# Zanue/EndoDAV

Hardware: AMD Instinct MI355X
Metric: depth frames/sec (518x518, T=8 clip) (higher is better)
Workload: dtype f32

## Files before the change

endodav_amd/csrc/conv_dma.hip:

```cpp
#include <atomic>
#include <cstdlib>
#include <type_traits>

#include "gemm_common.hpp"

namespace edv {
namespace {

constexpr int CBK = 32;
__device__ __attribute__((aligned(256))) float g_zero_page[64];

template <int WGM, int EP, bool SPLIT, bool BUF>
__global__ __launch_bounds__(256, 4) void conv3_dma_kernel(const GemmDesc g, const GemmSplit sp) {
    constexpr int WGN = 4 / WGM;
    constexpr int BM = 32 * WGM, BN = 32 * WGN;
    constexpr int IA = BM / 32, IB = BN / 32;
    constexpr int STAGE = (BM + BN) * CBK;
    __shared__ __attribute__((aligned(16))) float smem[2 * STAGE];
    const int tid = threadIdx.x, lane = tid & 63, wave = tid >> 6, l31 = lane & 31, lh = lane >> 5;
    const int wave_s = __builtin_amdgcn_readfirstlane(wave);
    const bool prelu = g.pre_relu != 0;
    const int wm = wave / WGN, wn = wave % WGN;
    const int tiles_n = (g.N + BN - 1) / BN;
    const int bid = xcd_remap(blockIdx.x, gridDim.x);
    const unsigned a_bytes = BUF ? (unsigned)((g.M > 0 ? ((g.M - 1) / (g.cOH * g.cOW) + 1) : 0) * (long long)g.cH * g.cW * g.cC * 4) : 0u;
    const auto rA = __builtin_amdgcn_make_buffer_rsrc(const_cast<float *>(g.A), 0, a_bytes, 0x00020000);
    const auto rW = __builtin_amdgcn_make_buffer_rsrc(const_cast<float *>(g.W), 0, 0xffffffff, 0x00020000);
    const int srow = lane >> 3, spos = lane & 7;
    const float *zero = g_zero_page + spos * 4;
    const int opix = g.cOH * g.cOW;
    const int nkt = g.K / CBK;
    const int ra = wm * 32 + l31, rb = wn * 32 + l31;
    const int swa = (ra >> 1) & 7, swb = (rb >> 1) & 7;

    long long u = SPLIT ? (long long)bid * sp.chunk : 0;
    const long long u_end = SPLIT ? (u + sp.chunk < sp.units ? u + sp.chunk : sp.units) : 0;
    bool once = true;
    for (;;) {
        int tile, kt0, kt1, lt = 0;
        float *part = nullptr;
        if (SPLIT) {
            if (u >= u_end) break;
            lt = (int)(u / nkt);
            kt0 = (int)(u - (long long)lt * nkt);
            const long long left = u_end - u;
            kt1 = kt0 + left < nkt ? kt0 + (int)left : nkt;
            tile = lt;
            if (!(kt0 == 0 && kt1 == nkt)) part = split_slot<SPLIT_SLOT>(sp, bid, u);
            u += kt1 - kt0;
        } else {
            if (!once) break;
            once = false;
            tile = bid;
            kt0 = 0;
            kt1 = nkt;
        }
        const int tm = tile / tiles_n, tn = tile - tm * tiles_n;
        const long long m0 = (long long)tm * BM;
        const int n0 = tn * BN;

        const float *pa[IA];
        unsigned va[IA], vb[IB];
        int okmask[IA];
#pragma unroll
        for (int i = 0; i < IA; ++i) {
            const int r = (BM / 4) * wave + 8 * i + srow;
            const int c = spos ^ ((r >> 1) & 7);
            long long m = m0 + r;
            m = m < g.M ? m : g.M - 1;
            const long long f = BUF ? (long long)((unsigned)m / (unsigned)opix) : m / opix;
            const int p = BUF ? (int)((unsigned)m - (unsigned)f * (unsigned)opix) : (int)(m - f * opix);
            const int oy = p / g.cOW, ox = p - oy * g.cOW;
            const int iy0 = oy * g.cS - 1, ix0 = ox * g.cS - 1;
            pa[i] = g.A + ((f * g.cH + iy0) * (long long)g.cW + ix0) * g.cC + c * 4;
            va[i] = (unsigned)((((f * g.cH + iy0 + 1) * (long long)g.cW + ix0 + 1) * g.cC + c * 4) * 4);
            int mk = 0;
#pragma unroll
            for (int d = 0; d < 3; ++d) {
                if (iy0 + d >= 0 && iy0 + d < g.cH) mk |= 1 << d;
                if (ix0 + d >= 0 && ix0 + d < g.cW) mk |= 8 << d;
            }
            okmask[i] = mk;
        }
        const float *pb[IB];
#pragma unroll
        for (int i = 0; i < IB; ++i) {
            const int r = (BN / 4) * wave + 8 * i + srow;
            const int c = spos ^ ((r >> 1) & 7);
            int n = n0 + r;
            n = n < g.N ? n : g.N - 1;
            pb[i] = g.W + (long long)n * g.ldw + c * 4;
            vb[i] = (unsigned)(((long long)n * g.ldw + c * 4) * 4);
        }
        int n_c0, n_dy, n_dx;
        {
            const int k = kt0 * CBK, tap = k / g.cC;
            n_c0 = k - tap * g.cC;
            n_dy = tap / 3;
            n_dx = tap - n_dy * 3;
        }
        auto issue = [&](int kt, int st) {
            float *sA = smem + st * STAGE, *sB = sA + BM * CBK;
            const int k = kt * CBK;
            const int dy = n_dy, dx = n_dx, c0 = n_c0;
            n_c0 += CBK;
            if (n_c0 == g.cC) {
                n_c0 = 0;
                if (++n_dx == 3) {
                    n_dx = 0;
                    ++n_dy;
                }
            }
            const long long off = ((long long)dy * g.cW + dx) * g.cC + c0;
            const int need = (1 << dy) | (8 << dx);
#pragma unroll
            for (int i = 0; i < IA; ++i) {
                if constexpr (BUF) {
                    const int delta = (((dy - 1) * g.cW + (dx - 1)) * g.cC) * 4;
                    const unsigned vo = (okmask[i] & need) == need ? va[i] + (unsigned)delta : 0x80000000u + a_bytes;
                    __builtin_amdgcn_raw_ptr_buffer_load_lds(rA, (__attribute__((address_space(3))) void *)(sA + ((BM / 4) * wave_s + 8 * i) * CBK), 16, (unsigned)vo,
                                                             (int)(c0 * 4), 0, 0);
                } else {
                    const float *src = (okmask[i] & need) == need ? pa[i] + off : zero;
                    __builtin_amdgcn_global_load_lds((const __attribute__((address_space(1))) void *)src,
                                                     (__attribute__((address_space(3))) void *)(sA + ((BM / 4) * wave + 8 * i) * CBK), 16, 0, 0);
                }
            }
#pragma unroll
            for (int i = 0; i < IB; ++i) {
                if constexpr (BUF)
                    __builtin_amdgcn_raw_ptr_buffer_load_lds(rW, (__attribute__((address_space(3))) void *)(sB + ((BN / 4) * wave_s + 8 * i) * CBK), 16, (unsigned)vb[i], (int)(k * 4), 0,
                                                             0);
                else
                    __builtin_amdgcn_global_load_lds((const __attribute__((address_space(1))) void *)(pb[i] + k),
                                                     (__attribute__((address_space(3))) void *)(sB + ((BN / 4) * wave + 8 * i) * CBK), 16, 0, 0);
            }
        };
        const float *fpa[4], *fpb[4];
#pragma unroll
        for (int q = 0; q < 4; ++q) {
            fpa[q] = smem + ra * CBK + (((2 * q + lh) ^ swa) << 2);
            fpb[q] = smem + BM * CBK + rb * CBK + (((2 * q + lh) ^ swb) << 2);
        }

        EpiCols<1> cols;
        if (EP != 0) cols = gemm_epilogue_prefetch<1>(g, n0, wn * 32, l31);
        float w2v = 0.f, b2v = 0.f;
        if constexpr (EP >= 8) {
            w2v = g.w2[n0 + l31 < g.N ? n0 + l31 : g.N - 1];
            if (g.b2) b2v = g.b2[0];
        }
        f32x16 acc[1][1];
        auto epilogue = [&]() {
            if constexpr (EP >= 8) {
                static_assert(EP < 8 || (WGM == 4 && BUF && !SPLIT), "the fused 1x1 needs every column of a row in one wave, and 32-bit offsets");
                gemm_epilogue_dot<EP - 8>(g, acc[0][0], cols, w2v, b2v, m0 + wave_s * 32, n0, l31, lh);
            } else if constexpr (BUF && EP >= 1 && EP <= 3)
                gemm_epilogue_buf<EP - 1>(g, acc[0][0], cols, m0 + (wave_s / WGN) * 32, n0 + (wave_s % WGN) * 32, l31, lh);
            else
                gemm_epilogue_ep<1, 1, STORE_ROWS, EP>(g, acc, cols, m0, n0, wm * 32, wn * 32, l31, lh);
        };
#pragma unroll
        for (int r = 0; r < 16; ++r) acc[0][0][r] = 0.f;

        issue(kt0, 0);
        asm volatile("s_waitcnt vmcnt(0)" ::: "memory");
        __builtin_amdgcn_s_barrier();
        auto ktile = [&](int kt, auto st_tag) {
            constexpr int ST = decltype(st_tag)::value;
            if (kt + 1 < kt1) issue(kt + 1, ST ^ 1);
            f32x4 fa[4], fb[4];
#pragma unroll
            for (int q = 0; q < 4; ++q) {
                fa[q] = *reinterpret_cast<const f32x4 *>(fpa[q] + ST * STAGE);
                fb[q] = *reinterpret_cast<const f32x4 *>(fpb[q] + ST * STAGE);
            }
            __builtin_amdgcn_sched_barrier(0);
            if (prelu) {
#pragma unroll
                for (int q = 0; q < 4; ++q)
#pragma unroll
                    for (int e = 0; e < 4; ++e) fa[q][e] = __builtin_amdgcn_fmed3f(fa[q][e], 0.f, __builtin_inff());
            }
#pragma unroll
            for (int q = 0; q < 4; ++q) {
#pragma unroll
                for (int e = 0; e < 4; ++e) acc[0][0] = __builtin_amdgcn_mfma_f32_32x32x2f32(fa[q][e], fb[q][e], acc[0][0], 0, 0, 0);
            }
            __builtin_amdgcn_sched_barrier(0);
            asm volatile("s_waitcnt vmcnt(0)" ::: "memory");
            asm volatile("s_waitcnt lgkmcnt(0)" ::: "memory");
            __builtin_amdgcn_s_barrier();
        };
        {
            int kt = kt0;
            for (; kt + 1 < kt1; kt += 2) {
                ktile(kt, std::integral_constant<int, 0>{});
                ktile(kt + 1, std::integral_constant<int, 1>{});
            }
            if (kt < kt1) ktile(kt, std::integral_constant<int, 0>{});
        }
        if (SPLIT && part) {
#pragma unroll
            for (int r = 0; r < 16; ++r) __hip_atomic_store(&part[(wave * 16 + r) * 64 + lane], acc[0][0][r], __ATOMIC_RELAXED, __HIP_MEMORY_SCOPE_AGENT);
            const long long ub = (long long)lt * nkt;
            int g0, g1;
            const bool last = split_handoff(sp, &sp.cnt[lt], ub, nkt, reinterpret_cast<int *>(smem), tid, g0, g1);
            if (last) {
#pragma unroll
                for (int r = 0; r < 16; ++r) acc[0][0][r] = 0.f;
                const float *base = sp.ws + (wave * 16) * 64 + lane;
                int gg = g0;
                for (; gg + 1 <= g1; gg += 2) {
                    const float *qa = split_piece<SPLIT_SLOT>(base, sp, gg, ub);
                    const float *qb = split_piece<SPLIT_SLOT>(base, sp, gg + 1, ub);
                    float ta[16], tb[16];
#pragma unroll
                    for (int r = 0; r < 16; ++r) {
                        ta[r] = __hip_atomic_load(qa + r * 64, __ATOMIC_RELAXED, __HIP_MEMORY_SCOPE_AGENT);
                        tb[r] = __hip_atomic_load(qb + r * 64, __ATOMIC_RELAXED, __HIP_MEMORY_SCOPE_AGENT);
                    }
#pragma unroll
                    for (int r = 0; r < 16; ++r) acc[0][0][r] = (acc[0][0][r] + ta[r]) + tb[r];
                }
                if (gg <= g1) {
                    const float *qa = split_piece<SPLIT_SLOT>(base, sp, gg, ub);
#pragma unroll
                    for (int r = 0; r < 16; ++r) acc[0][0][r] += __hip_atomic_load(qa + r * 64, __ATOMIC_RELAXED, __HIP_MEMORY_SCOPE_AGENT);
                }
                epilogue();
            }
        } else {
            epilogue();
        }
    }
}

template <int WGM, int EP, bool SPLIT>
void launch_variant(const GemmDesc &d, const GemmSplit &sp, bool buf, unsigned grid, hipStream_t st) {
    if (buf) EDV_LAUNCH((conv3_dma_kernel<WGM, EP, SPLIT, true>), dim3(grid), dim3(256), 0, st, d, sp);
    else EDV_LAUNCH((conv3_dma_kernel<WGM, EP, SPLIT, false>), dim3(grid), dim3(256), 0, st, d, sp);
}

template <int WGM, int EP>
int conv_slots() {
    static DeviceSlotCache cache;
    return resident_workgroups(cache, (const void *)conv3_dma_kernel<WGM, EP, true, true>, 256, 0, 4, nullptr, nullptr);
}

template <int WGM, int EP>
int launch_conv_ep(const GemmDesc &d, long long tiles, hipStream_t st) {
    static const bool split_on = env_int("EDV_CONV_SPLIT", 1) != 0;
    static const bool buf_off = env_int("EDV_CONV_BUF", 1) == 0;
    const long long frames = (d.M - 1) / ((long long)d.cOH * d.cOW) + 1;
    const long long ld_out = std::max(std::max(d.ldc, d.R1 ? d.ldr1 : 0), d.R2 ? d.ldr2 : 0);
    const bool buf = !buf_off && frames * d.cH * d.cW * d.cC * 4 < (1ll << 31) - (1 << 20) && (long long)d.N * d.ldw * 4 < (1ll << 32) - (1 << 20) &&
                     (d.M + 64) * ld_out * 4 < (1ll << 32) - 4096;
    const SplitPolicy &pol = conv_dma_split_policy();
    GemmSplit sp{};
    long long grid;
    plan_plain(tiles, pol, &sp, &grid);
    if (split_on && d.ws && plan_split(tiles, conv_slots<WGM, EP>(), d.K / CBK, pol, &sp, &grid)) {
        split_bind(&sp, d.ws, pol);
        if (split_ws_floats(sp, pol) <= d.ws_floats && (uintptr_t)d.ws % 16 == 0) {
            launch_variant<WGM, EP, true>(d, sp, buf, (unsigned)grid, st);
            EDV_LAUNCH_OK();
            return 0;
        }
        grid = tiles;
    }
    launch_variant<WGM, EP, false>(d, sp, buf, (unsigned)grid, st);
    EDV_LAUNCH_OK();
    return 0;
}

template <int WGM>
int launch_conv(const GemmDesc &d, hipStream_t st) {
    constexpr int BM = 32 * WGM, BN = 32 * (4 / WGM);
    const long long tiles = ((d.M + BM - 1) / BM) * (long long)((d.N + BN - 1) / BN);
    EDV_CHECK(tiles > 0 && tiles < (1ll << 31), "bad grid");
    switch (epilogue_kind(d)) {
        case 1: return launch_conv_ep<WGM, 1>(d, tiles, st);
        case 3: return launch_conv_ep<WGM, 3>(d, tiles, st);
        default: return launch_conv_ep<WGM, 0>(d, tiles, st);
    }
}

std::atomic<int> g_conv_impl{0};

bool dot_fits_buffer(const GemmDesc &d) {
    const long long frames = (d.M - 1) / ((long long)d.cOH * d.cOW) + 1;
    return frames * d.cH * d.cW * d.cC * 4 < (1ll << 31) - (1 << 20) && (long long)d.N * d.ldw * 4 < (1ll << 32) - (1 << 20) && (d.M + 128) * 4 < (1ll << 32) - (1 << 20);
}

template <int EP>
int launch_conv_dot(const GemmDesc &d, hipStream_t st) {
    const long long tiles = (d.M + 127) / 128;
    EDV_CHECK(tiles > 0 && tiles < (1ll << 31), "bad grid");
    GemmSplit sp{};
    long long grid;
    plan_plain(tiles, conv_dma_split_policy(), &sp, &grid);
    EDV_LAUNCH((conv3_dma_kernel<4, EP, false, true>), dim3((unsigned)grid), dim3(256), 0, st, d, sp);
    EDV_LAUNCH_OK();
    return 0;
}

}

void set_conv_impl(int mode) { g_conv_impl.store(mode < 0 || mode > 2 ? 0 : mode, std::memory_order_relaxed); }
int conv_impl() { return g_conv_impl.load(std::memory_order_relaxed); }
bool conv_dot_enabled() {
    return conv_impl() != 1 && env_int("EDV_CONV_DOT", 1) != 0;
}

const SplitPolicy &conv_dma_split_policy() {
    static const SplitPolicy p{.min_kt = 18, .min_tiles = 16, .max_rounds = 0, .widen = false, .counters = SPLIT_MAX_COUNTERS, .slot_floats = SPLIT_SLOT,
                               .whole_rounds = false, .deep_kt = 48, .idle_factor = 8};
    return p;
}

bool conv_dma_supported(const GemmDesc &d) {
    return d.loader == LOAD_CONV3 && d.store == STORE_ROWS && d.cC % CBK == 0 && d.K == 9 * d.cC && d.ldw % 4 == 0 && d.M > 0 && d.N > 0;
}

bool conv_dot_supported(const GemmDesc &d) {
    return conv_dma_supported(d) && d.N <= 32 && (d.act == ACT_NONE || d.act == ACT_RELU) && d.act2 != ACT_GELU && d.act2 >= ACT_NONE && d.act2 <= ACT_SIGMOID_NEG &&
           !d.gamma && !d.R1 && !d.R2 && !d.P1 && d.c_map.period == 0 && dot_fits_buffer(d);
}

int conv_dot(const GemmDesc &d, hipStream_t st) {
    EDV_CHECK(d.A && d.W && d.w2 && d.dot_out, "null operand");
    EDV_CHECK(conv_dot_supported(d), "fused 1x1 epilogue: Cin % 32 == 0, Cout <= 32, post-activation none / ReLU, no residual, operands below 2 GB");
    EDV_CHECK(((uintptr_t)d.A % 16 == 0) && ((uintptr_t)d.W % 16 == 0), "A/W must be 16-byte aligned");
    if (conv_halo_wanted(d)) return conv_halo(d, st);
    return d.act == ACT_RELU ? launch_conv_dot<8 + ACT_RELU>(d, st) : launch_conv_dot<8 + ACT_NONE>(d, st);
}

int conv_dma(const GemmDesc &d, hipStream_t st) {
    EDV_CHECK(d.A && d.W && d.C, "null operand");
    EDV_CHECK(conv_dma_supported(d), "LDS-DMA convolution needs Cin % 32 == 0");
    EDV_CHECK(((uintptr_t)d.A % 16 == 0) && ((uintptr_t)d.W % 16 == 0), "A/W must be 16-byte aligned");
    if (conv_halo_wanted(d)) return conv_halo(d, st);
    return d.N <= 32 ? launch_conv<4>(d, st) : launch_conv<2>(d, st);
}

}
```

endodav_amd/csrc/conv_halo.hip:

```cpp
#include <cstdlib>
#include <type_traits>

#include "gemm_common.hpp"

namespace edv {
namespace {

constexpr int HBK = 32;
constexpr int TH = 8, TW = 16;
constexpr int ROW_BYTES = 3 * 64 * 16;
constexpr int PIX_BYTES = 9 * 16;
constexpr int PLANE_BYTES = (TH + 2) * ROW_BYTES;
constexpr int WSTAGE = 32 * HBK;
constexpr unsigned LANE_OUT = 0x80000000u;
constexpr unsigned ROW_OUT = 0x7ff00000u;

template <int NCB, int ACT, bool DOT>
__global__ __launch_bounds__(256, NCB == 1 ? 4 : 2) void conv3_halo_kernel(const GemmDesc g) {
    __shared__ __attribute__((aligned(16))) float smem[2 * WSTAGE + NCB * PLANE_BYTES / 4];
    constexpr int CIN = NCB * 32, NKT = 9 * NCB;
    const int tid = threadIdx.x, lane = tid & 63, l31 = lane & 31, lh = lane >> 5;
    const int wave_s = __builtin_amdgcn_readfirstlane(tid >> 6);
    const bool prelu = g.pre_relu != 0;
    const int H = g.cH, W = g.cW;
    const int bid = xcd_remap(blockIdx.x, gridDim.x);
    const int tiles_x = (W + TW - 1) / TW, tiles_y = (H + TH - 1) / TH;
    const int f = bid / (tiles_x * tiles_y), tr = bid - f * (tiles_x * tiles_y);
    const int ty = tr / tiles_x, tx = tr - ty * tiles_x;
    const int oy0 = ty * TH, ox0 = tx * TW;
    const int frames = (int)(g.M / ((long long)H * W));
    const unsigned a_bytes = (unsigned)((long long)frames * H * W * CIN * 4);
    const auto rA = __builtin_amdgcn_make_buffer_rsrc(const_cast<float *>(g.A), 0, a_bytes, 0x00020000);
    const auto rW = __builtin_amdgcn_make_buffer_rsrc(const_cast<float *>(g.W), 0, 0xffffffff, 0x00020000);
    float *const sW = smem;
    char *const patch = reinterpret_cast<char *>(smem + 2 * WSTAGE);

    unsigned pat[3];
#pragma unroll
    for (int k = 0; k < 3; ++k) {
        const unsigned ci = (unsigned)(k * 64 + lane);
        const unsigned hx = ci / 9u, c = ci - 9u * hx;
        const int ix = ox0 - 1 + (int)hx;
        pat[k] = (hx < (unsigned)(TW + 2) && c < 8u && ix >= 0 && ix < W) ? (unsigned)((ix * CIN + (int)c * 4) * 4) : LANE_OUT;
    }
#pragma unroll
    for (int t = 0; t < ((TH + 2) * NCB + 3) / 4; ++t) {
        const int u = wave_s + 4 * t;
        if (u < (TH + 2) * NCB) {
            const int cb = NCB == 1 ? 0 : u / (TH + 2), hy = u - cb * (TH + 2);
            const int iy = oy0 - 1 + hy;
            const unsigned so = (iy >= 0 && iy < H) ? (unsigned)((((f * H + iy) * W) * CIN + cb * 32) * 4) : ROW_OUT;
            char *dst = patch + cb * PLANE_BYTES + hy * ROW_BYTES;
#pragma unroll
            for (int k = 0; k < 3; ++k)
                __builtin_amdgcn_raw_ptr_buffer_load_lds(rA, (__attribute__((address_space(3))) void *)(dst + k * 1024), 16, (unsigned)pat[k], (int)so, 0, 0);
        }
    }
    const int srow = lane >> 3, spos = lane & 7;
    unsigned vb;
    {
        const int r = 8 * wave_s + srow;
        const int c = spos ^ ((r >> 1) & 7);
        const int n = r < g.N ? r : g.N - 1;
        vb = (unsigned)((n * g.ldw + c * 4) * 4);
    }
    auto issue_w = [&](int kt, int stg) {
        __builtin_amdgcn_raw_ptr_buffer_load_lds(rW, (__attribute__((address_space(3))) void *)(sW + stg * WSTAGE + 8 * wave_s * HBK), 16, (unsigned)vb, (int)(kt * HBK * 4),
                                                 0, 0);
    };
    const int swb = (l31 >> 1) & 7;
    const float *fpb[4];
#pragma unroll
    for (int q = 0; q < 4; ++q) fpb[q] = sW + l31 * HBK + (((2 * q + lh) ^ swb) << 2);
    const char *const a0 = patch + (2 * wave_s) * ROW_BYTES + (l31 >> 4) * ROW_BYTES + (l31 & 15) * PIX_BYTES + lh * 16;

    EpiCols<1> cols = gemm_epilogue_prefetch<1>(g, 0, 0, l31);
    float w2v = 0.f, b2v = 0.f;
    if constexpr (DOT) {
        w2v = g.w2[l31 < g.N ? l31 : g.N - 1];
        if (g.b2) b2v = g.b2[0];
    }
    f32x16 acc;
#pragma unroll
    for (int r = 0; r < 16; ++r) acc[r] = 0.f;

    issue_w(0, 0);
    asm volatile("s_waitcnt vmcnt(0)" ::: "memory");
    __builtin_amdgcn_s_barrier();
#pragma unroll
    for (int kt = 0; kt < NKT; ++kt) {
        const int stg = kt & 1, tap = kt / NCB, cb = kt - tap * NCB, dy = tap / 3, dx = tap - 3 * dy;
        if (kt + 1 < NKT) issue_w(kt + 1, stg ^ 1);
        f32x4 fa[4], fb[4];
#pragma unroll
        for (int q = 0; q < 4; ++q) {
            fa[q] = *reinterpret_cast<const f32x4 *>(a0 + cb * PLANE_BYTES + dy * ROW_BYTES + dx * PIX_BYTES + q * 32);
            fb[q] = *reinterpret_cast<const f32x4 *>(fpb[q] + stg * WSTAGE);
        }
        __builtin_amdgcn_sched_barrier(0);
        if (prelu) {
#pragma unroll
            for (int q = 0; q < 4; ++q)
#pragma unroll
                for (int e = 0; e < 4; ++e) fa[q][e] = __builtin_amdgcn_fmed3f(fa[q][e], 0.f, __builtin_inff());
        }
#pragma unroll
        for (int q = 0; q < 4; ++q) {
#pragma unroll
            for (int e = 0; e < 4; ++e) acc = __builtin_amdgcn_mfma_f32_32x32x2f32(fa[q][e], fb[q][e], acc, 0, 0, 0);
        }
        __builtin_amdgcn_sched_barrier(0);
        asm volatile("s_waitcnt vmcnt(0)" ::: "memory");
        asm volatile("s_waitcnt lgkmcnt(0)" ::: "memory");
        __builtin_amdgcn_s_barrier();
    }

    const int oyw = oy0 + 2 * wave_s;
    const unsigned mbase = (unsigned)((f * H + oyw) * W + ox0);
    if constexpr (DOT) {
        const float v = gemm_dot_reduce<ACT>(g, acc, cols, w2v, b2v, l31 < g.N, l31);
        const int i = l31 & 15, r = 2 * i + (l31 >> 4);
        const int py = r >> 3, px = (r & 3) + 8 * ((r >> 2) & 1) + 4 * lh;
        const bool ok = i < 8 && oyw + py < H && ox0 + px < W;
        const auto ro = __builtin_amdgcn_make_buffer_rsrc(g.dot_out, 0, (int)(unsigned)(g.M * 4), 0x00020000);
        __builtin_amdgcn_raw_buffer_store_b32(__float_as_uint(v), ro, (int)(ok ? (unsigned)((py * W + px) * 4) : LANE_OUT), (int)(mbase * 4u), EDV_EPI_STORE_AUX);
    } else {
        using f32x2 = __attribute__((ext_vector_type(2))) float;
        const int ld = g.ldc;
        const unsigned lane_off = l31 >= g.N ? LANE_OUT : (unsigned)((4 * lh * ld + l31) * 4);
        const int lim = W - ox0 - 4 * lh;
        unsigned vo[8];
#pragma unroll
        for (int j = 0; j < 8; ++j) vo[j] = ((j & 3) + 8 * (j >> 2)) < lim ? lane_off : LANE_OUT;
        unsigned so[16];
#pragma unroll
        for (int r = 0; r < 16; ++r)
            so[r] = oyw + (r >> 3) < H ? (mbase + (unsigned)((r >> 3) * W + (r & 3) + 8 * ((r >> 2) & 1))) * (unsigned)(ld * 4) : ROW_OUT;
        f32x2 res[8];
#pragma unroll
        for (int i = 0; i < 8; ++i) res[i] = f32x2{0.f, 0.f};
        const int bytes = (int)(unsigned)(g.M * ld * 4);
        if (g.R1) {
            const auto rs = __builtin_amdgcn_make_buffer_rsrc(const_cast<float *>(g.R1), 0, bytes, 0x00020000);
#pragma unroll
            for (int r = 0; r < 16; ++r) res[r >> 1][r & 1] = __uint_as_float(__builtin_amdgcn_raw_buffer_load_b32(rs, (int)vo[(r & 3) + 4 * ((r >> 2) & 1)], (int)so[r], 0));
        }
        if (g.R2) {
            const auto rs = __builtin_amdgcn_make_buffer_rsrc(const_cast<float *>(g.R2), 0, bytes, 0x00020000);
#pragma unroll
            for (int r = 0; r < 16; ++r) res[r >> 1][r & 1] += __uint_as_float(__builtin_amdgcn_raw_buffer_load_b32(rs, (int)vo[(r & 3) + 4 * ((r >> 2) & 1)], (int)so[r], 0));
        }
        const auto rc = __builtin_amdgcn_make_buffer_rsrc(g.C, 0, bytes, 0x00020000);
        const f32x2 bias = {cols.bias[0], cols.bias[0]}, gam = {cols.gam[0], cols.gam[0]};
#pragma unroll
        for (int i = 0; i < 8; ++i) {
            f32x2 v = f32x2{acc[2 * i], acc[2 * i + 1]} + bias;
            if (ACT == ACT_RELU) v = f32x2{fmaxf(v[0], 0.0f), fmaxf(v[1], 0.0f)};
            v = v * gam + res[i];
#pragma unroll
            for (int e = 0; e < 2; ++e) {
                const int r = 2 * i + e;
                const float ve = e ? v[1] : v[0];
                __builtin_amdgcn_raw_buffer_store_b32(__float_as_uint(ve), rc, (int)vo[(r & 3) + 4 * ((r >> 2) & 1)], (int)so[r], EDV_EPI_STORE_AUX);
            }
        }
    }
}

template <int NCB, int ACT>
int launch_halo(const GemmDesc &d, unsigned grid, hipStream_t st) {
    if (d.w2) EDV_LAUNCH((conv3_halo_kernel<NCB, ACT, true>), dim3(grid), dim3(256), 0, st, d);
    else EDV_LAUNCH((conv3_halo_kernel<NCB, ACT, false>), dim3(grid), dim3(256), 0, st, d);
    EDV_LAUNCH_OK();
    return 0;
}

long long halo_tiles(const GemmDesc &d) { return (d.M / ((long long)d.cH * d.cW)) * ((d.cH + TH - 1) / TH) * (long long)((d.cW + TW - 1) / TW); }

}

bool conv_halo_supported(const GemmDesc &d) {
    if (!conv_dma_supported(d) || d.cS != 1 || d.N > 32 || (d.cC != 32 && d.cC != 64)) return false;
    if (d.M % ((long long)d.cH * d.cW) != 0 || halo_tiles(d) >= (1ll << 31)) return false;
    const long long lim = (1ll << 31) - (1 << 20);
    if (d.M * d.cC * 4 >= lim || (long long)d.N * d.ldw * 4 >= lim) return false;
    if (d.w2) return d.M * 4 < lim;
    const int ep = epilogue_kind(d);
    if (ep != 1 + ACT_NONE && ep != 1 + ACT_RELU) return false;
    if ((d.R1 && d.ldr1 != d.ldc) || (d.R2 && d.ldr2 != d.ldc)) return false;
    return d.M * d.ldc * 4 < lim;
}

bool conv_halo_pays(const GemmDesc &d) { return (d.cC == 32 || d.cC == 64) && d.N <= 32 && halo_tiles(d) >= 4096; }

bool conv_halo_wanted(const GemmDesc &d) {
    if (conv_impl() == 1 || !conv_halo_supported(d) || env_int("EDV_CONV_HALO", 1) == 0) return false;
    return conv_impl() == 2 || conv_halo_pays(d);
}

int conv_halo(const GemmDesc &d, hipStream_t st) {
    EDV_CHECK(d.A && d.W && (d.w2 ? (const void *)d.dot_out : (const void *)d.C), "null operand");
    EDV_CHECK(conv_halo_supported(d), "halo convolution: stride 1, Cin 32 or 64, Cout <= 32, operands below 2 GB");
    EDV_CHECK(((uintptr_t)d.A % 16 == 0) && ((uintptr_t)d.W % 16 == 0), "A/W must be 16-byte aligned");
    const unsigned grid = (unsigned)halo_tiles(d);
    const bool relu = d.act == ACT_RELU;
    if (d.cC == 32) return relu ? launch_halo<1, ACT_RELU>(d, grid, st) : launch_halo<1, ACT_NONE>(d, grid, st);
    return relu ? launch_halo<2, ACT_RELU>(d, grid, st) : launch_halo<2, ACT_NONE>(d, grid, st);
}

}
```

endodav_amd/csrc/ops.hpp:

```cpp
#pragma once
#include "common.hpp"
#include "streamk_plan.hpp"

namespace edv {

enum { ACT_NONE = 0, ACT_GELU = 1, ACT_RELU = 2, ACT_SIGMOID = 3, ACT_SIGMOID_NEG = 4 };
enum { LOAD_DENSE = 0, LOAD_CONV3 = 1 };
enum { STORE_ROWS = 0, STORE_SHUFFLE = 1 };

struct GemmDesc {
    const float *A = nullptr;
    int lda = 0;
    RowMap a_map{0, 0, 0};
    const float *W = nullptr;
    int ldw = 0;
    float *C = nullptr;
    int ldc = 0;
    RowMap c_map{0, 0, 0};
    long long M = 0;
    int N = 0, K = 0;
    const float *bias = nullptr;
    int act = ACT_NONE;
    const float *gamma = nullptr;
    const float *R1 = nullptr;
    int ldr1 = 0;
    RowMap r1_map{0, 0, 0};
    const float *R2 = nullptr;
    int ldr2 = 0;
    const float *P1 = nullptr;
    int ldp1 = 0;
    RowMap p1_map{0, 0, 0};
    int loader = LOAD_DENSE;
    int cH = 0, cW = 0, cC = 0, cOH = 0, cOW = 0, cS = 1, pre_relu = 0;
    int store = STORE_ROWS;
    int geglu = 0;
    int ps_s = 0, ps_C = 0, ps_h = 0, ps_w = 0;
    float *ws = nullptr;
    size_t ws_floats = 0;
    const void *Wx6 = nullptr;
    const float *w2 = nullptr, *b2 = nullptr;
    float *dot_out = nullptr;
    int act2 = ACT_NONE;
};
int gemm(const GemmDesc &d, hipStream_t st);
size_t gemm_x6_planes_bytes(int N, int K);
int gemm_x6_split(const float *W, void *planes, int N, int K, hipStream_t st);
bool gemm_x6_supported(const GemmDesc &d);
int gemm_x6(const GemmDesc &d, hipStream_t st);
size_t gemm_workspace();
size_t gemm_counter_bytes();
bool gemm_dma_supported(const GemmDesc &d);
bool gemm_geglu_supported(const GemmDesc &d);
int pack_geglu(const float *w, const float *b, float *wi, float *bi, int N, int K, hipStream_t st);
int gemm_dma(const GemmDesc &d, hipStream_t st);
bool conv_dma_supported(const GemmDesc &d);
int conv_dma(const GemmDesc &d, hipStream_t st);
bool conv_dot_supported(const GemmDesc &d);
int conv_dot(const GemmDesc &d, hipStream_t st);
bool conv_halo_supported(const GemmDesc &d);
bool conv_halo_wanted(const GemmDesc &d);
int conv_halo(const GemmDesc &d, hipStream_t st);
void set_conv_impl(int mode);
int conv_impl();
bool conv_dot_enabled();
const SplitPolicy &gemm_dma_split_policy();
const SplitPolicy &gemm_x6_split_policy();
const SplitPolicy &conv_dma_split_policy();
const char *gemm_kernel_name(const GemmDesc &d);

size_t attn_spatial_workspace(int F, int N, int heads, bool x6 = false);
int attn_spatial(const float *qkv, float *out, int F, int N, int heads, float *ws, size_t ws_floats, hipStream_t st, float *lse = nullptr, bool x6 = false);
size_t attn_spatial_bwd_workspace(int F, int N, int heads);
int attn_spatial_bwd(const float *qkv, const float *out, const float *dout, const float *lse, float *delta, float *dqkv, int F, int N, int heads, float *ws,
                     size_t ws_floats, hipStream_t st);
int attn_temporal(const float *qkv, float *out, int B, int T, int P, int C, int heads, hipStream_t st);
int geglu(const float *x, float *y, long long M, int inner, hipStream_t st);
int rope_qk(float *qkv, const float *table, int B, int T, int P, int C, bool transpose, hipStream_t st);

int layernorm(const float *x, RowMap in_map, const float *w, const float *b, float *y, RowMap out_map, long long rows, int dim,
              float eps, const float *pe, int rows_per_frame, int T, hipStream_t st, int act = ACT_NONE, bool accumulate = false);
size_t groupnorm_workspace(int F, int P, int C);
int groupnorm(const float *x, const float *w, const float *b, float *y, float *stats, int F, int P, int C, int groups, float eps, hipStream_t st,
              float *part = nullptr, size_t part_floats = 0);

int patchify(const float *x, float *cols, int F, int H, int W, int ih, int iw, hipStream_t st, int ld = 588)  ;
int bilinear(const float *x, float *y, int F, int H, int W, int C, int OH, int OW, int act, hipStream_t st, const float *add = nullptr);
int dot_channels(const float *x, const float *w, const float *b, float *y, long long M, int C, int act, hipStream_t st);
int cls_rows(const float *cls, const float *pos, float *tokens, int F, int ntok, int D, hipStream_t st);
int sigmoid_inplace(float *x, long long n, hipStream_t st);
int resize_bicubic(const float *x, float *y, int NP, int H, int W, int OH, int OW, hipStream_t st);
int ingest_u8(const uint8_t *src, int src_frames, const int32_t *slots_host, int n, float *out, int H, int W, int OH, int OW, hipStream_t st);
size_t stitch_workspace();
int stitch_fit(const float *disp, int ih, int iw, const float *tail, int fh, int fw, float *st, void *ws, size_t ws_bytes, hipStream_t stream);
int stitch_apply(const float *disp, int ih, int iw, const float *st, float *tail, float *out_new, int fh, int fw, hipStream_t stream);
size_t metrics_workspace(long long n, int h, int w);
int masked_median(const float *x, const float *gate, long long count, float lo, float hi, double *out, void *ws, size_t ws_bytes, hipStream_t stream);
int metrics_pred(const float *disp, const float *gt, float *pred, long long n, int h, int w, double min_depth, double max_depth, int align, float factor, float cap,
                 double *scal, void *ws, size_t ws_bytes, hipStream_t stream);
int metrics_errors(const float *pred, const float *gt, long long n, int h, int w, float cap, double *out, void *ws, size_t ws_bytes, hipStream_t stream);
int metrics_temporal(const float *pred, const float *gt, long long n, int h, int w, float cap, const double *mats, double *out, float *warp, void *ws,
                     size_t ws_bytes, hipStream_t stream);
size_t render_workspace(long long n);
int render_range(const float *x, long long n, int h, int w, int mode, long long rank_lo, long long rank_hi, float *range, void *ws, size_t ws_bytes, hipStream_t stream);
int render_colorize(const float *x, long long n, int h, int w, const float *range, int range_stride, float eps, int clip, const uint8_t *lut, const uint8_t *beside,
                    uint8_t *out, hipStream_t stream);
struct CloudSel {
    const float *x;
    long long n;
    int h, w, step, mode;
    float lo, span, gain, near_z, far_z;
    const uint8_t *mask;
    long long mask_stride;
};
int cloud_tile_pixels();
size_t cloud_workspace(long long n, int h, int w, int step);
int cloud_count(const CloudSel &s, long long *offsets, void *ws, size_t ws_bytes, hipStream_t stream);
int cloud_scatter(const CloudSel &s, const double *cams, int cam_stride, const uint8_t *frames, const long long *offsets, const void *ws, size_t ws_bytes,
                  float *points, uint8_t *colors, long long capacity, hipStream_t stream);
int bicubic_pos(const float *grid, float *out, int S, int D, int oh, int ow, float scale_h, float scale_w, hipStream_t st);

int pack_conv3x3(const float *w, float *out, int Cout, int Cin, hipStream_t st);
int pack_convT(const float *w, float *wout, const float *b, float *bout, int Cin, int Cout, int s, hipStream_t st);
int copy_f32(const float *src, float *dst, long long n, hipStream_t st);
int fold_lora(const float *W, const float *A, const float *B, const float *U, const float *V, float scale, float *out, int nout, int nin,
              int r, hipStream_t st);
int fold_ssb(const float *W, const float *a, const float *b, float *out, int nout, int nin, hipStream_t st);
int fold_bn(float *w, const float *b, const float *gamma, const float *beta, const float *mean, const float *var, float eps, float *bout, int nout, int K,
            hipStream_t st);
int fold_dash(const float *Utop, const float *idx, const float *Vtop, float *inout, int nout, int nin, int r, hipStream_t st);

int layernorm_bwd(const float *x, RowMap xmap, const float *w, const float *dy, RowMap dymap, float *dx, RowMap dxmap, long long rows, int dim, float eps,
                  bool accumulate, hipStream_t st);
int ew_bwd(const float *d, const float *src, const float *add, float *out, long long n, int mode, hipStream_t st);
int sigmoid_bwd(const float *g, const float *s, float *out, long long n, hipStream_t st);
int geglu_bwd(const float *x, const float *dy, float *dx, long long M, int inner, hipStream_t st);
int transpose_scale(const float *W, int ldw, const float *gamma, float *Wt, int N, int K, hipStream_t st);
int skinny_xwt(const float *X, long long M, int K, int ldx, const float *Wr, int r, float *T, hipStream_t st);
constexpr int TALL_SPLITS = 64;
size_t tall_tn_workspace(int N, int r);
int tall_tn(const float *Y, int ldy, const float *T, long long M, int N, int r, float scale, const float *rowscale, float *part, float *out, hipStream_t st);
int lora_grad_finalize(const float *dBp, const float *dApT, const float *A, const float *Bm, const float *U, const float *V, float *dA, float *dB, float *dU,
                       float *dV, int nout, int nin, int r, hipStream_t st);
size_t lora_grads_workspace(long long M, int nin, int nout, int r);
int lora_grads(const float *X, int ldx, const float *G, int ldg, long long M, int nin, int nout, int r, const float *A, const float *Bm, const float *U,
               const float *V, float s, const float *gamma, float *ws, size_t ws_floats, float *dA, float *dB, float *dU, float *dV, hipStream_t st);
int ssb_prep(const float *W, const float *a, const float *b, const float *gamma, float *Wa, float *gb, int nout, int nin, hipStream_t st);
int col_dot(const float *P, const float *Q, long long M, int N, const float *scale, float *part, float *out, hipStream_t st);
int bilinear_bwd(const float *dy, float *dx, int F, int ih, int iw, int C, int oh, int ow, bool accumulate, hipStream_t st);
int dot_channels_bwd(const float *g, const float *disp, const float *w, const float *o2, float *d_o2, float *gz_out, long long npix, int C, int mode,
                     hipStream_t st);
size_t conv3_wgrad_workspace(int F, int H, int W, int Cin, int Cout);
int conv3_wgrad(const float *x, const float *dy, float *dw, int F, int H, int W, int Cin, int Cout, float *ws, size_t ws_floats, bool accumulate,
                hipStream_t st);
size_t colsum_workspace(int N);
int colsum_rows(const float *P, const float *rowscale, long long M, int N, float *ws, size_t ws_floats, float *out, bool accumulate, hipStream_t st);
constexpr int CS_MAX_JOBS = 16, CS_MAX_OUTS = 48, CS_MAX_PARTS = 64;
struct ColsumJob {
    const float *src = nullptr;
    long long ld = 0, rows = 0, chunk = 0;
    RowMap map{0, 0, 0};
    int N = 0, parts = 0, cw_log = 0;
    float *slab = nullptr;
};
struct ColsumOut {
    const float *slab;
    int rows, N;
    const float *scale;
    float *dst;
    int accumulate;
};
ColsumJob colsum_job(const float *src, long long ld, long long rows, RowMap map, int N);
int colsum_stage1_launch(const ColsumJob *jobs, int n, hipStream_t st);
int colsum_stage2_launch(const ColsumOut *outs, int n, hipStream_t st);
size_t colsum_batch_workspace(int n, const long long *rows, const int *cols);
int colsum_batch(int n, const float *const *src, const long long *ld, const long long *rows, const RowMap *maps, const int *cols, const float *const *scale,
                 float *const *dst, const int *accumulate, float *ws, size_t ws_floats, hipStream_t st);
int groupnorm_bwd(const float *x, const float *stats, const float *w, const float *dy, float *sums, float *dx, int F, int P, int C, int groups, bool accumulate,
                  hipStream_t st);
int attn_temporal_bwd(const float *qkv, const float *dout, float *dqkv, int B, int T, int P, int C, int heads, hipStream_t st);
int pixel_unshuffle(const float *dy, float *A, int F, int h, int w, int C, int s, hipStream_t st);
int conv3x3_s2_bwd(const float *dy, const float *wpacked, float *dx, int F, int H, int W, int Cin, int Cout, hipStream_t st);
int dilate2(const float *dy, float *z, int F, int H, int W, int C, hipStream_t st);
int pack_conv3x3_bwd(const float *w, float *out, int Cout, int Cin, hipStream_t st);

struct TrainerLossIn {
    const float *color[4];
    const float *color_nb[2];
    const float *K, *invK;
    const float *T[2];
    const float *refined[4][2], *registration[4][2], *transform[4][2];
    const float *mask[2];
    const float *position[4][2];
    const float *disp[4];
    int disp_h[4], disp_w[4];
};
struct TrainerLossW {
    float disparity_smoothness, transform_constraint, transform_smoothness, depth_reproj, depth_flow;
    int tune_temporal;
    float min_depth, max_depth;
};
struct TrainerLossGrads {
    float *disp[4];
    float *refined[4][2], *transform[4][2];
    float *K, *invK, *T[2];
};
size_t trainer_loss_workspace(int N, int H, int W);
int trainer_loss(const TrainerLossIn &in, int N, int H, int W, const TrainerLossW &w, float *losses, const TrainerLossGrads &g, float *ws, size_t ws_floats, hipStream_t st);
size_t photometric_loss_workspace(int B, int T, int H, int W);
int photometric_loss(const float *frames, const float *const disp[4], const int *dh, const int *dw, int B, int T, int H, int W, const float *K, const float *invK,
                     const float *Tprev, const float *Tnext, float min_depth, float max_depth, float smoothness, float *loss, float *const grad[4], float *ws,
                     size_t ws_floats, hipStream_t st);

}
```

Baseline: 1106.

## Extend halo 3x3 convolution to 64 output channels with two column blocks

The halo-tiled 3x3 convolution kernel gains an NB template parameter, so each workgroup computes two 32-wide output-column blocks against the same LDS input patch, reusing the staged activations. Convs with Cout up to 64 can now use the halo path. The router picks it only when the DMA conv would not use split-K, which adds a planning call per dispatch. The two-block variant doubles accumulators and weight staging, lowering occupancy (launch bounds 3 instead of 4 for Cin 32).

```diff
diff --git a/endodav_amd/csrc/conv_dma.hip b/endodav_amd/csrc/conv_dma.hip
--- a/endodav_amd/csrc/conv_dma.hip
+++ b/endodav_amd/csrc/conv_dma.hip
@@ -249,8 +249,19 @@
 }
 
 template <int WGM, int EP>
+bool conv_plan_split(const GemmDesc &d, long long tiles, GemmSplit *sp, long long *grid) {
+    static const bool split_on = env_int("EDV_CONV_SPLIT", 1) != 0;
+    return split_on && d.ws && plan_split(tiles, conv_slots<WGM, EP>(), d.K / CBK, conv_dma_split_policy(), sp, grid);
+}
+
+template <int WGM>
+long long conv_tiles(const GemmDesc &d) {
+    constexpr int BM = 32 * WGM, BN = 32 * (4 / WGM);
+    return ((d.M + BM - 1) / BM) * (long long)((d.N + BN - 1) / BN);
+}
+
+template <int WGM, int EP>
 int launch_conv_ep(const GemmDesc &d, long long tiles, hipStream_t st) {
-    static const bool split_on = env_int("EDV_CONV_SPLIT", 1) != 0;
     static const bool buf_off = env_int("EDV_CONV_BUF", 1) == 0;
     const long long frames = (d.M - 1) / ((long long)d.cOH * d.cOW) + 1;
     const long long ld_out = std::max(std::max(d.ldc, d.R1 ? d.ldr1 : 0), d.R2 ? d.ldr2 : 0);
@@ -260,7 +271,7 @@
     GemmSplit sp{};
     long long grid;
     plan_plain(tiles, pol, &sp, &grid);
-    if (split_on && d.ws && plan_split(tiles, conv_slots<WGM, EP>(), d.K / CBK, pol, &sp, &grid)) {
+    if (conv_plan_split<WGM, EP>(d, tiles, &sp, &grid)) {
         split_bind(&sp, d.ws, pol);
         if (split_ws_floats(sp, pol) <= d.ws_floats && (uintptr_t)d.ws % 16 == 0) {
             launch_variant<WGM, EP, true>(d, sp, buf, (unsigned)grid, st);
@@ -276,8 +287,7 @@
 
 template <int WGM>
 int launch_conv(const GemmDesc &d, hipStream_t st) {
-    constexpr int BM = 32 * WGM, BN = 32 * (4 / WGM);
-    const long long tiles = ((d.M + BM - 1) / BM) * (long long)((d.N + BN - 1) / BN);
+    const long long tiles = conv_tiles<WGM>(d);
     EDV_CHECK(tiles > 0 && tiles < (1ll << 31), "bad grid");
     switch (epilogue_kind(d)) {
         case 1: return launch_conv_ep<WGM, 1>(d, tiles, st);
@@ -323,6 +333,19 @@
     return d.loader == LOAD_CONV3 && d.store == STORE_ROWS && d.cC % CBK == 0 && d.K == 9 * d.cC && d.ldw % 4 == 0 && d.M > 0 && d.N > 0;
 }
 
+bool conv_dma_splits(const GemmDesc &d) {
+    if (!conv_dma_supported(d)) return false;
+    GemmSplit sp{};
+    long long grid = 0;
+    const int ek = epilogue_kind(d);
+    if (d.N <= 32) {
+        const long long t = conv_tiles<4>(d);
+        return ek == 1 ? conv_plan_split<4, 1>(d, t, &sp, &grid) : ek == 3 ? conv_plan_split<4, 3>(d, t, &sp, &grid) : conv_plan_split<4, 0>(d, t, &sp, &grid);
+    }
+    const long long t = conv_tiles<2>(d);
+    return ek == 1 ? conv_plan_split<2, 1>(d, t, &sp, &grid) : ek == 3 ? conv_plan_split<2, 3>(d, t, &sp, &grid) : conv_plan_split<2, 0>(d, t, &sp, &grid);
+}
+
 bool conv_dot_supported(const GemmDesc &d) {
     return conv_dma_supported(d) && d.N <= 32 && (d.act == ACT_NONE || d.act == ACT_RELU) && d.act2 != ACT_GELU && d.act2 >= ACT_NONE && d.act2 <= ACT_SIGMOID_NEG &&
            !d.gamma && !d.R1 && !d.R2 && !d.P1 && d.c_map.period == 0 && dot_fits_buffer(d);
diff --git a/endodav_amd/csrc/conv_halo.hip b/endodav_amd/csrc/conv_halo.hip
--- a/endodav_amd/csrc/conv_halo.hip
+++ b/endodav_amd/csrc/conv_halo.hip
@@ -11,12 +11,14 @@
 constexpr int ROW_BYTES = 3 * 64 * 16;
 constexpr int PIX_BYTES = 9 * 16;
 constexpr int PLANE_BYTES = (TH + 2) * ROW_BYTES;
-constexpr int WSTAGE = 32 * HBK;
+constexpr int WBLOCK = 32 * HBK;
 constexpr unsigned LANE_OUT = 0x80000000u;
 constexpr unsigned ROW_OUT = 0x7ff00000u;
 
-template <int NCB, int ACT, bool DOT>
-__global__ __launch_bounds__(256, NCB == 1 ? 4 : 2) void conv3_halo_kernel(const GemmDesc g) {
+template <int NCB, int NB, int ACT, bool DOT>
+__global__ __launch_bounds__(256, NCB == 1 ? (NB == 1 ? 4 : 3) : 2) void conv3_halo_kernel(const GemmDesc g) {
+    static_assert(NB == 1 || !DOT, "the fused 1x1 needs every column of a row in one lane group");
+    constexpr int WSTAGE = NB * WBLOCK;
     __shared__ __attribute__((aligned(16))) float smem[2 * WSTAGE + NCB * PLANE_BYTES / 4];
     constexpr int CIN = NCB * 32, NKT = 9 * NCB;
     const int tid = threadIdx.x, lane = tid & 63, l31 = lane & 31, lh = lane >> 5;
@@ -57,16 +59,19 @@
         }
     }
     const int srow = lane >> 3, spos = lane & 7;
-    unsigned vb;
-    {
-        const int r = 8 * wave_s + srow;
+    unsigned vb[NB];
+#pragma unroll
+    for (int i = 0; i < NB; ++i) {
+        const int r = 8 * NB * wave_s + 8 * i + srow;
         const int c = spos ^ ((r >> 1) & 7);
         const int n = r < g.N ? r : g.N - 1;
-        vb = (unsigned)((n * g.ldw + c * 4) * 4);
+        vb[i] = (unsigned)((n * g.ldw + c * 4) * 4);
     }
     auto issue_w = [&](int kt, int stg) {
-        __builtin_amdgcn_raw_ptr_buffer_load_lds(rW, (__attribute__((address_space(3))) void *)(sW + stg * WSTAGE + 8 * wave_s * HBK), 16, (unsigned)vb, (int)(kt * HBK * 4),
-                                                 0, 0);
+#pragma unroll
+        for (int i = 0; i < NB; ++i)
+            __builtin_amdgcn_raw_ptr_buffer_load_lds(rW, (__attribute__((address_space(3))) void *)(sW + stg * WSTAGE + (8 * NB * wave_s + 8 * i) * HBK), 16, (unsigned)vb[i],
+                                                     (int)(kt * HBK * 4), 0, 0);
     };
     const int swb = (l31 >> 1) & 7;
     const float *fpb[4];
@@ -74,15 +79,19 @@
     for (int q = 0; q < 4; ++q) fpb[q] = sW + l31 * HBK + (((2 * q + lh) ^ swb) << 2);
     const char *const a0 = patch + (2 * wave_s) * ROW_BYTES + (l31 >> 4) * ROW_BYTES + (l31 & 15) * PIX_BYTES + lh * 16;
 
-    EpiCols<1> cols = gemm_epilogue_prefetch<1>(g, 0, 0, l31);
+    EpiCols<1> cols[NB];
+#pragma unroll
+    for (int j = 0; j < NB; ++j) cols[j] = gemm_epilogue_prefetch<1>(g, 0, 32 * j, l31);
     float w2v = 0.f, b2v = 0.f;
     if constexpr (DOT) {
         w2v = g.w2[l31 < g.N ? l31 : g.N - 1];
         if (g.b2) b2v = g.b2[0];
     }
-    f32x16 acc;
-#pragma unroll
-    for (int r = 0; r < 16; ++r) acc[r] = 0.f;
+    f32x16 acc[NB];
+#pragma unroll
+    for (int j = 0; j < NB; ++j)
+#pragma unroll
+        for (int r = 0; r < 16; ++r) acc[j][r] = 0.f;
 
     issue_w(0, 0);
     asm volatile("s_waitcnt vmcnt(0)" ::: "memory");
@@ -91,12 +100,16 @@
     for (int kt = 0; kt < NKT; ++kt) {
         const int stg = kt & 1, tap = kt / NCB, cb = kt - tap * NCB, dy = tap / 3, dx = tap - 3 * dy;
         if (kt + 1 < NKT) issue_w(kt + 1, stg ^ 1);
-        f32x4 fa[4], fb[4];
+        f32x4 fa[4], fb[NB][4];
 #pragma unroll
         for (int q = 0; q < 4; ++q) {
             fa[q] = *reinterpret_cast<const f32x4 *>(a0 + cb * PLANE_BYTES + dy * ROW_BYTES + dx * PIX_BYTES + q * 32);
-            fb[q] = *reinterpret_cast<const f32x4 *>(fpb[q] + stg * WSTAGE);
-        }
+            fb[0][q] = *reinterpret_cast<const f32x4 *>(fpb[q] + stg * WSTAGE);
+        }
+#pragma unroll
+        for (int j = 1; j < NB; ++j)
+#pragma unroll
+            for (int q = 0; q < 4; ++q) fb[j][q] = *reinterpret_cast<const f32x4 *>(fpb[q] + stg * WSTAGE + j * WBLOCK);
         __builtin_amdgcn_sched_barrier(0);
         if (prelu) {
 #pragma unroll
@@ -105,9 +118,12 @@
                 for (int e = 0; e < 4; ++e) fa[q][e] = __builtin_amdgcn_fmed3f(fa[q][e], 0.f, __builtin_inff());
         }
 #pragma unroll
-        for (int q = 0; q < 4; ++q) {
-#pragma unroll
-            for (int e = 0; e < 4; ++e) acc = __builtin_amdgcn_mfma_f32_32x32x2f32(fa[q][e], fb[q][e], acc, 0, 0, 0);
+        for (int j = 0; j < NB; ++j) {
+#pragma unroll
+            for (int q = 0; q < 4; ++q) {
+#pragma unroll
+                for (int e = 0; e < 4; ++e) acc[j] = __builtin_amdgcn_mfma_f32_32x32x2f32(fa[q][e], fb[j][q][e], acc[j], 0, 0, 0);
+            }
         }
         __builtin_amdgcn_sched_barrier(0);
         asm volatile("s_waitcnt vmcnt(0)" ::: "memory");
@@ -118,7 +134,7 @@
     const int oyw = oy0 + 2 * wave_s;
     const unsigned mbase = (unsigned)((f * H + oyw) * W + ox0);
     if constexpr (DOT) {
-        const float v = gemm_dot_reduce<ACT>(g, acc, cols, w2v, b2v, l31 < g.N, l31);
+        const float v = gemm_dot_reduce<ACT>(g, acc[0], cols[0], w2v, b2v, l31 < g.N, l31);
         const int i = l31 & 15, r = 2 * i + (l31 >> 4);
         const int py = r >> 3, px = (r & 3) + 8 * ((r >> 2) & 1) + 4 * lh;
         const bool ok = i < 8 && oyw + py < H && ox0 + px < W;
@@ -127,64 +143,84 @@
     } else {
         using f32x2 = __attribute__((ext_vector_type(2))) float;
         const int ld = g.ldc;
-        const unsigned lane_off = l31 >= g.N ? LANE_OUT : (unsigned)((4 * lh * ld + l31) * 4);
+        const unsigned lane_off0 = l31 >= g.N ? LANE_OUT : (unsigned)((4 * lh * ld + l31) * 4);
         const int lim = W - ox0 - 4 * lh;
-        unsigned vo[8];
-#pragma unroll
-        for (int j = 0; j < 8; ++j) vo[j] = ((j & 3) + 8 * (j >> 2)) < lim ? lane_off : LANE_OUT;
+        unsigned vo0[8];
+#pragma unroll
+        for (int j = 0; j < 8; ++j) vo0[j] = ((j & 3) + 8 * (j >> 2)) < lim ? lane_off0 : LANE_OUT;
         unsigned so[16];
 #pragma unroll
         for (int r = 0; r < 16; ++r)
             so[r] = oyw + (r >> 3) < H ? (mbase + (unsigned)((r >> 3) * W + (r & 3) + 8 * ((r >> 2) & 1))) * (unsigned)(ld * 4) : ROW_OUT;
-        f32x2 res[8];
-#pragma unroll
-        for (int i = 0; i < 8; ++i) res[i] = f32x2{0.f, 0.f};
         const int bytes = (int)(unsigned)(g.M * ld * 4);
-        if (g.R1) {
-            const auto rs = __builtin_amdgcn_make_buffer_rsrc(const_cast<float *>(g.R1), 0, bytes, 0x00020000);
-#pragma unroll
-            for (int r = 0; r < 16; ++r) res[r >> 1][r & 1] = __uint_as_float(__builtin_amdgcn_raw_buffer_load_b32(rs, (int)vo[(r & 3) + 4 * ((r >> 2) & 1)], (int)so[r], 0));
-        }
-        if (g.R2) {
-            const auto rs = __builtin_amdgcn_make_buffer_rsrc(const_cast<float *>(g.R2), 0, bytes, 0x00020000);
-#pragma unroll
-            for (int r = 0; r < 16; ++r) res[r >> 1][r & 1] += __uint_as_float(__builtin_amdgcn_raw_buffer_load_b32(rs, (int)vo[(r & 3) + 4 * ((r >> 2) & 1)], (int)so[r], 0));
-        }
-        const auto rc = __builtin_amdgcn_make_buffer_rsrc(g.C, 0, bytes, 0x00020000);
-        const f32x2 bias = {cols.bias[0], cols.bias[0]}, gam = {cols.gam[0], cols.gam[0]};
-#pragma unroll
-        for (int i = 0; i < 8; ++i) {
-            f32x2 v = f32x2{acc[2 * i], acc[2 * i + 1]} + bias;
-            if (ACT == ACT_RELU) v = f32x2{fmaxf(v[0], 0.0f), fmaxf(v[1], 0.0f)};
-            v = v * gam + res[i];
-#pragma unroll
-            for (int e = 0; e < 2; ++e) {
-                const int r = 2 * i + e;
-                const float ve = e ? v[1] : v[0];
-                __builtin_amdgcn_raw_buffer_store_b32(__float_as_uint(ve), rc, (int)vo[(r & 3) + 4 * ((r >> 2) & 1)], (int)so[r], EDV_EPI_STORE_AUX);
-            }
-        }
-    }
-}
-
-template <int NCB, int ACT>
+#pragma unroll
+        for (int nb = 0; nb < NB; ++nb) {
+            unsigned vo[8];
+#pragma unroll
+            for (int j = 0; j < 8; ++j) vo[j] = nb == 0 ? vo0[j] : (32 * nb + l31 >= g.N ? LANE_OUT : vo0[j] + (unsigned)(128 * nb));
+            f32x2 res[8];
+#pragma unroll
+            for (int i = 0; i < 8; ++i) res[i] = f32x2{0.f, 0.f};
+            if (g.R1) {
+                const auto rs = __builtin_amdgcn_make_buffer_rsrc(const_cast<float *>(g.R1), 0, bytes, 0x00020000);
+#pragma unroll
+                for (int r = 0; r < 16; ++r)
+                    res[r >> 1][r & 1] = __uint_as_float(__builtin_amdgcn_raw_buffer_load_b32(rs, (int)vo[(r & 3) + 4 * ((r >> 2) & 1)], (int)so[r], 0));
+            }
+            if (g.R2) {
+                const auto rs = __builtin_amdgcn_make_buffer_rsrc(const_cast<float *>(g.R2), 0, bytes, 0x00020000);
+#pragma unroll
+                for (int r = 0; r < 16; ++r)
+                    res[r >> 1][r & 1] += __uint_as_float(__builtin_amdgcn_raw_buffer_load_b32(rs, (int)vo[(r & 3) + 4 * ((r >> 2) & 1)], (int)so[r], 0));
+            }
+            const auto rc = __builtin_amdgcn_make_buffer_rsrc(g.C, 0, bytes, 0x00020000);
+            const f32x2 bias = {cols[nb].bias[0], cols[nb].bias[0]}, gam = {cols[nb].gam[0], cols[nb].gam[0]};
+#pragma unroll
+            for (int i = 0; i < 8; ++i) {
+                f32x2 v = f32x2{acc[nb][2 * i], acc[nb][2 * i + 1]} + bias;
+                if (ACT == ACT_RELU) v = f32x2{fmaxf(v[0], 0.0f), fmaxf(v[1], 0.0f)};
+                v = v * gam + res[i];
+#pragma unroll
+                for (int e = 0; e < 2; ++e) {
+                    const int r = 2 * i + e;
+                    const float ve = e ? v[1] : v[0];
+                    __builtin_amdgcn_raw_buffer_store_b32(__float_as_uint(ve), rc, (int)vo[(r & 3) + 4 * ((r >> 2) & 1)], (int)so[r], EDV_EPI_STORE_AUX);
+                }
+            }
+        }
+    }
+}
+
+template <int NCB, int NB, int ACT>
 int launch_halo(const GemmDesc &d, unsigned grid, hipStream_t st) {
-    if (d.w2) EDV_LAUNCH((conv3_halo_kernel<NCB, ACT, true>), dim3(grid), dim3(256), 0, st, d);
-    else EDV_LAUNCH((conv3_halo_kernel<NCB, ACT, false>), dim3(grid), dim3(256), 0, st, d);
+    if constexpr (NB == 1) {
+        if (d.w2) {
+            EDV_LAUNCH((conv3_halo_kernel<NCB, 1, ACT, true>), dim3(grid), dim3(256), 0, st, d);
+            EDV_LAUNCH_OK();
+            return 0;
+        }
+    }
+    EDV_LAUNCH((conv3_halo_kernel<NCB, NB, ACT, false>), dim3(grid), dim3(256), 0, st, d);
     EDV_LAUNCH_OK();
     return 0;
 }
 
+template <int NCB>
+void halo64_report_slots() {
+    static DeviceSlotCache cache;
+    resident_workgroups(cache, (const void *)conv3_halo_kernel<NCB, 2, ACT_NONE, false>, 256, 0, 0, nullptr, NCB == 1 ? "conv3_halo_kernel<1,2,...>" : "conv3_halo_kernel<2,2,...>");
+}
+
 long long halo_tiles(const GemmDesc &d) { return (d.M / ((long long)d.cH * d.cW)) * ((d.cH + TH - 1) / TH) * (long long)((d.cW + TW - 1) / TW); }
 
 }
 
 bool conv_halo_supported(const GemmDesc &d) {
-    if (!conv_dma_supported(d) || d.cS != 1 || d.N > 32 || (d.cC != 32 && d.cC != 64)) return false;
+    if (!conv_dma_supported(d) || d.cS != 1 || d.N > 64 || (d.cC != 32 && d.cC != 64)) return false;
     if (d.M % ((long long)d.cH * d.cW) != 0 || halo_tiles(d) >= (1ll << 31)) return false;
     const long long lim = (1ll << 31) - (1 << 20);
     if (d.M * d.cC * 4 >= lim || (long long)d.N * d.ldw * 4 >= lim) return false;
-    if (d.w2) return d.M * 4 < lim;
+    if (d.w2) return d.N <= 32 && d.M * 4 < lim;
     const int ep = epilogue_kind(d);
     if (ep != 1 + ACT_NONE && ep != 1 + ACT_RELU) return false;
     if ((d.R1 && d.ldr1 != d.ldc) || (d.R2 && d.ldr2 != d.ldc)) return false;
@@ -195,17 +231,27 @@
 
 bool conv_halo_wanted(const GemmDesc &d) {
     if (conv_impl() == 1 || !conv_halo_supported(d) || env_int("EDV_CONV_HALO", 1) == 0) return false;
-    return conv_impl() == 2 || conv_halo_pays(d);
+    if (conv_impl() != 2 && !conv_halo_pays(d)) return false;
+    return d.N <= 32 || !conv_dma_splits(d);
 }
 
 int conv_halo(const GemmDesc &d, hipStream_t st) {
     EDV_CHECK(d.A && d.W && (d.w2 ? (const void *)d.dot_out : (const void *)d.C), "null operand");
-    EDV_CHECK(conv_halo_supported(d), "halo convolution: stride 1, Cin 32 or 64, Cout <= 32, operands below 2 GB");
+    EDV_CHECK(conv_halo_supported(d), "halo convolution: stride 1, Cin 32 or 64, Cout <= 64 (<= 32 with the fused 1x1), operands below 2 GB");
     EDV_CHECK(((uintptr_t)d.A % 16 == 0) && ((uintptr_t)d.W % 16 == 0), "A/W must be 16-byte aligned");
     const unsigned grid = (unsigned)halo_tiles(d);
     const bool relu = d.act == ACT_RELU;
-    if (d.cC == 32) return relu ? launch_halo<1, ACT_RELU>(d, grid, st) : launch_halo<1, ACT_NONE>(d, grid, st);
-    return relu ? launch_halo<2, ACT_RELU>(d, grid, st) : launch_halo<2, ACT_NONE>(d, grid, st);
-}
-
-}
+    if (d.N <= 32) {
+        if (d.cC == 32) return relu ? launch_halo<1, 1, ACT_RELU>(d, grid, st) : launch_halo<1, 1, ACT_NONE>(d, grid, st);
+        return relu ? launch_halo<2, 1, ACT_RELU>(d, grid, st) : launch_halo<2, 1, ACT_NONE>(d, grid, st);
+    }
+    static const bool report = getenv("EDV_DEBUG_SLOTS") != nullptr;
+    if (d.cC == 32) {
+        if (report) halo64_report_slots<1>();
+        return relu ? launch_halo<1, 2, ACT_RELU>(d, grid, st) : launch_halo<1, 2, ACT_NONE>(d, grid, st);
+    }
+    if (report) halo64_report_slots<2>();
+    return relu ? launch_halo<2, 2, ACT_RELU>(d, grid, st) : launch_halo<2, 2, ACT_NONE>(d, grid, st);
+}
+
+}
diff --git a/endodav_amd/csrc/ops.hpp b/endodav_amd/csrc/ops.hpp
--- a/endodav_amd/csrc/ops.hpp
+++ b/endodav_amd/csrc/ops.hpp
@@ -55,6 +55,7 @@
 int gemm_dma(const GemmDesc &d, hipStream_t st);
 bool conv_dma_supported(const GemmDesc &d);
 int conv_dma(const GemmDesc &d, hipStream_t st);
+bool conv_dma_splits(const GemmDesc &d);
 bool conv_dot_supported(const GemmDesc &d);
 int conv_dot(const GemmDesc &d, hipStream_t st);
 bool conv_halo_supported(const GemmDesc &d);
diff --git a/scratch/kb_conv_halo64.py b/scratch/kb_conv_halo64.py
--- /dev/null
+++ b/scratch/kb_conv_halo64.py
@@ -0,0 +1,97 @@
+import ctypes as C
+import math
+import os
+import sys
+
+import torch
+
+sys.path.insert(0, os.path.dirname(os.path.dirname(os.path.abspath(__file__))))
+from endodav_amd import _lib
+
+lib = _lib.load()
+cuda = torch.device("cuda:0")
+REPS, ROUNDS = 30, 4
+Fr, Cin, Cout = 8, 64, 64
+
+
+def st():
+    return C.c_void_p(torch.cuda.current_stream().cuda_stream)
+
+
+def rnd(*shape, seed=0, scale=1.0):
+    g = torch.Generator().manual_seed(seed)
+    return ((torch.rand(*shape, generator=g) * 2 - 1) * scale).to(cuda)
+
+
+def timed(fn):
+    for _ in range(5):
+        fn()
+    torch.cuda.synchronize()
+    a, b = torch.cuda.Event(enable_timing=True), torch.cuda.Event(enable_timing=True)
+    a.record()
+    for _ in range(REPS):
+        fn()
+    b.record()
+    torch.cuda.synchronize()
+    return a.elapsed_time(b) / REPS * 1e3
+
+
+def timed_cold(fn, flush):
+    ts = []
+    for _ in range(12):
+        flush.fill_(1.0)
+        a, b = torch.cuda.Event(enable_timing=True), torch.cuda.Event(enable_timing=True)
+        a.record()
+        fn()
+        b.record()
+        torch.cuda.synchronize()
+        ts.append(a.elapsed_time(b) * 1e3)
+    ts = sorted(ts[2:])
+    return ts[len(ts) // 2]
+
+
+def run(S):
+    x = rnd(Fr, S, S, Cin, seed=1)
+    w = rnd(Cout, Cin, 3, 3, seed=2, scale=1 / math.sqrt(9 * Cin))
+    b = rnd(Cout, seed=3, scale=0.1)
+    r1, r2 = rnd(Fr, S, S, Cout, seed=4), rnd(Fr, S, S, Cout, seed=5)
+    wp = torch.empty(Cout * 9 * Cin, device=cuda)
+    _lib.check(lib.edv_pack_conv3x3(w.data_ptr(), wp.data_ptr(), Cout, Cin, st()))
+    y = torch.empty((Fr, S, S, Cout), device=cuda)
+
+    def conv_relu():
+        _lib.check(lib.edv_conv3x3(x.data_ptr(), wp.data_ptr(), b.data_ptr(), y.data_ptr(), Fr, S, S, Cin, Cout, 1, 1, 1, None, None, st()))
+
+    def conv_res():
+        _lib.check(lib.edv_conv3x3(x.data_ptr(), wp.data_ptr(), b.data_ptr(), y.data_ptr(), Fr, S, S, Cin, Cout, 1, 1, 0, r1.data_ptr(), r2.data_ptr(), st()))
+
+    patches = Fr * ((S + 7) // 8) * ((S + 15) // 16)
+    for form, fn in (("pre_relu+relu", conv_relu), ("pre_relu+R1+R2", conv_res)):
+        outs = {}
+        res = {"dma": [], "halo": []}
+        for _ in range(ROUNDS):
+            for vname, mode in (("dma", 1), ("halo", 2)):
+                _lib.check(lib.edv_set_conv_impl(mode))
+                res[vname].append(round(timed(fn), 1))
+                outs[vname] = y.clone()
+        _lib.check(lib.edv_set_conv_impl(0))
+        same = torch.equal(outs["dma"], outs["halo"])
+        warm_d, warm_h = res["dma"][1:], res["halo"][1:]
+        verdict = "halo faster in every warm round" if max(warm_h) < min(warm_d) else "NOT faster in every warm round"
+        gflop = 2.0 * Fr * S * S * 9 * Cin * Cout / 1e9
+        print(f"64->64 {Fr}x{S}x{S} ({patches} patches, {gflop:.2f} GFLOP) {form:15s} dma {res['dma']}  halo {res['halo']}  "
+              f"warm means {sum(warm_d) / 3:.1f} / {sum(warm_h) / 3:.1f} us ({gflop / (sum(warm_h) / 3) * 1e3:.1f} TFLOP/s halo)  {verdict}  bits equal: {same}", flush=True)
+        if COLD:
+            cold = {}
+            for _ in range(2):
+                for vname, mode in (("dma", 1), ("halo", 2)):
+                    _lib.check(lib.edv_set_conv_impl(mode))
+                    cold.setdefault(vname, []).append(round(timed_cold(fn, FLUSH), 1))
+            _lib.check(lib.edv_set_conv_impl(0))
+            print(f"       cold launches (median of ten behind a 512 MB fill, two alternations): dma {cold['dma']}  halo {cold['halo']}", flush=True)
+
+
+COLD = "cold" in sys.argv[1:]
+FLUSH = torch.empty(128 * 1024 * 1024, device=cuda) if COLD else None
+for S in [int(a) for a in sys.argv[1:] if a != "cold"] or [148, 74, 37, 19]:
+    run(S)
```

Result: no change. 1107 (median of 2 runs) (+0.0%).
